# WeeFav/Visual-Odometry-GPU

Measured on AMD Instinct MI355X. Metric: ORB detect+describe frames/sec (1241x376, 8 lvls), higher is better.
Workload: dtype u8; 1 GPU; KITTI-shaped 1241x376 u8, 8 levels s=1.2, 1000 features, FAST-9 t=20, NMS 3x3, Harris top-N, blur5 all levels, BRIEF-256; batch=1024 frames/step/GPU resident in HBM (stream A); distinct_resident_batches=2, fast_early_exit=True, pyramid_blur_fused=True, pyramid_top_rows_first=True, pipelined_batches=True

## Files before the change

### visual-odometry-gpu_amd/csrc/orbx_kernels.hip

```cpp
#include <hip/hip_runtime.h>

#include <cstdlib>

#include "orbx_internal.h"
#include "orbx_math.h"
#include "orbx_wave.h"

__constant__ __attribute__((aligned(16))) int8_t c_pattern[1024] = {
#include "pattern_31.inc"
};


typedef uint16_t __attribute__((aligned(1))) u16_unaligned;

__device__ __forceinline__ void decode_tile(const OrbxTileMap& tm, int nlevels, int& l, int& tx, int& ty) {
  const int t = blockIdx.x;
  l = 0;
#pragma unroll 1
  for (int i = 1; i < nlevels; i++)
    if (t >= tm.begin[i]) l = i;
  const int local = t - tm.begin[l];
  ty = local / tm.tiles_x[l];
  tx = local - ty * tm.tiles_x[l];
}

__device__ __forceinline__ int reflect101(int p, int len) {
  if (p < 0) p = -p;
  if (p >= len) p = 2 * len - p - 2;
  p = p < 0 ? 0 : p;
  return p >= len ? len - 1 : p;
}

typedef uint32_t __attribute__((aligned(1))) u32_unaligned;
struct __attribute__((packed, aligned(1))) uint2_unaligned {
  uint32_t x, y;
  __device__ operator uint2() const { return make_uint2(x, y); }
};

template <int ROWS, bool WIN8>
__device__ __forceinline__ void pyr_rows(const uint8_t* __restrict__ src, int in_stride, int w0, int h0,
                                         const OrbxResizeTap* __restrict__ ytaps, int yb, int lh,
                                         const uint32_t (&ofs)[4], const uint32_t (&cc)[4],
                                         __amdgpu_buffer_rsrc_t rout, uint32_t voff_st, uint32_t vmask, int pitch) {
// ... 320 lines not shown
    for (int j = 0; j < K; j++) out[j] = pr[j] + 2.0f * pr[j + 1] + pr[j + 2];
  };
  float pr[3][P], hs[3][K];
  cvt_row(0, pr[0]);
  cvt_row(1, pr[1]);
  hsum(pr[0], hs[0]);
  hsum(pr[1], hs[1]);
  float a = 0.f, b = 0.f, c = 0.f;
#pragma unroll
  for (int i = 0; i < K; i++) {
    float(&p0)[P] = pr[i % 3];
    float(&p1)[P] = pr[(i + 1) % 3];
    float(&p2)[P] = pr[(i + 2) % 3];
    cvt_row(i + 2, p2);
    hsum(p2, hs[(i + 2) % 3]);
    float vs[P];
#pragma unroll
    for (int j = 0; j < P; j++) vs[j] = p0[j] + 2.0f * p1[j] + p2[j];
#pragma unroll
    for (int j = 0; j < K; j++) {
      const float gx = vs[j + 2] - vs[j];
      const float gy = hs[(i + 2) % 3][j] - hs[i % 3][j];
      const float wgt = g[i * K + j];
      a = __fadd_rn(a, __fmul_rn(__fmul_rn(gx, gx), wgt));
      c = __fadd_rn(c, __fmul_rn(__fmul_rn(gy, gy), wgt));
      b = __fadd_rn(b, __fmul_rn(__fmul_rn(gx, gy), wgt));
    }
  }
  const float det = __fsub_rn(__fmul_rn(a, c), __fmul_rn(b, b));
  const float trace = __fadd_rn(a, c);
  return __fsub_rn(det, __fmul_rn(__fmul_rn(kk, trace), trace));
}

__device__ __forceinline__ float harris_any(const uint8_t* img, int w, int h, int pitch, int x, int y,
                                            const float* __restrict__ g, int K, float kk) {
  const int m = K / 2 + 1;
  if (x >= m - 1 && y >= m - 1 && x <= w - m && y <= h - m && w >= 4 && h >= 4) {
    if (K == 7) return harris_fast<7>(img, w, h, pitch, x, y, g, kk);
    if (K == 5) return harris_fast<5>(img, w, h, pitch, x, y, g, kk);
    if (K == 3) return harris_fast<3>(img, w, h, pitch, x, y, g, kk);
  }
  return harris_at(img, w, h, pitch, x, y, g, K, kk);
}

template <int K, int RPL, int G>
__device__ __forceinline__ float harris_row_group(const uint8_t* img, int pitch, int x, int y,
                                                  const float* __restrict__ g, float kk, int sub) {
  constexpr int r = K / 2, P = K + 2, NR = RPL + 2;
  constexpr int NL = (K + RPL - 1) / RPL;
  const int row0 = (sub < NL ? sub : NL - 1) * RPL;
  const int xs = x - r - 1;
  const int a0 = xs & ~3, off = xs - a0;
  float p[NR][P];
#pragma unroll
  for (int i = 0; i < NR; i++) {
    const int pr = min(row0 + i, P - 1);
    const uint32_t* row = reinterpret_cast<const uint32_t*>(img + (size_t)(y - r - 1 + pr) * pitch + a0);
    const uint32_t d0 = row[0], d1 = row[1], d2 = row[2];
    const uint32_t q[3] = {__builtin_amdgcn_alignbyte(d1, d0, off), __builtin_amdgcn_alignbyte(d2, d1, off),
                           d2 >> (8 * off)};
#pragma unroll
    for (int j = 0; j < P; j++) p[i][j] = (float)((q[j >> 2] >> (8 * (j & 3))) & 0xffu);
  }
  float hs[NR][K];
#pragma unroll
  for (int i = 0; i < NR; i++)
#pragma unroll
    for (int j = 0; j < K; j++) hs[i][j] = p[i][j] + 2.0f * p[i][j + 1] + p[i][j + 2];
  float pa[RPL][K], pb[RPL][K], pc[RPL][K];
#pragma unroll
// ... 63 lines not shown
      last = (5 + RPL - 1) / RPL - 1;
    } else {
      v = harris_row_group<3, RPL, G>(img, pitch, xx, yy, g, kk, sub);
      last = (3 + RPL - 1) / RPL - 1;
    }
    if (active && fast && sub == last) {
      res = v;
      writer = true;
    }
  }
  if (active && !fast && sub == 0) {
    res = harris_at(img, w, h, pitch, x, y, g, K, kk);
    writer = true;
  }
  return res;
}

__global__ __launch_bounds__(256) void k_harris2_flat(const uint8_t* __restrict__ img, int w, int h, int pitch,
                                                      const orbx_keypoint* __restrict__ kps, int nkp,
                                                      const float* __restrict__ gauss, int K, float kk,
                                                      float* __restrict__ resp) {
  constexpr int G = 8, RPL = 1;
  const int j = blockIdx.x * 32 + (threadIdx.x >> 3), sub = threadIdx.x & 7;
  const bool active = j < nkp;
  orbx_keypoint kp = {4, 4};
  if (active) kp = kps[j];
  bool writer;
  const float v = harris_group<RPL, G>(img, w, h, pitch, kp.x, kp.y, gauss, K, kk, sub, active, writer);
  if (writer) resp[j] = v;
}


#define LVL_THREADS 512
__global__ __launch_bounds__(LVL_THREADS) __attribute__((amdgpu_waves_per_eu(4, 8))) void k_level_select(OrbxPlan plan, int mode, const u64* __restrict__ mask,
                                                              const uint8_t* __restrict__ pyr,
                                                              const float* __restrict__ gauss, int K, float kk,
                                                              orbx_keypoint* __restrict__ sel_lkp,
                                                              float* __restrict__ sel_resp,
                                                              int32_t* __restrict__ sel_count,
                                                              uint32_t* __restrict__ need) {
  extern __shared__ __attribute__((aligned(16))) unsigned char s_dyn[];
  __shared__ int s_wsum[4][LVL_THREADS / 64];
  const int f = blockIdx.x, l = blockIdx.y;
  const OrbxLevel& L = plan.L[l];
  const int cap = L.cap, cap2 = (cap + 1) & ~1;
  u64* s_key = reinterpret_cast<u64*>(s_dyn);
  uint32_t* s_kp = reinterpret_cast<uint32_t*>(s_dyn + 8 * (size_t)cap2);
  float* s_r = reinterpret_cast<float*>(s_dyn + 12 * (size_t)cap2);
  const u64* m = mask + (size_t)f * plan.mask_words + L.mask_off;
  const int nwords = L.h * L.mask_wpr;
  const int tid = threadIdx.x, lane = tid & 63, wave = tid >> 6;

  int base = 0;
  for (int w0 = 0; w0 < nwords && base < cap; w0 += 4 * LVL_THREADS) {
    u64 v[4];
#pragma unroll
    for (int q = 0; q < 4; q++) {
      const int i = w0 + LVL_THREADS * q + tid;
      v[q] = i < nwords ? m[i] : 0ull;
    }
    int incl[4], c[4];
#pragma unroll
    for (int q = 0; q < 4; q++) {
      c[q] = __popcll(v[q]);
      incl[q] = wave_scan_incl(c[q]);
      if (lane == 63) s_wsum[q][wave] = incl[q];
    }
    __syncthreads();
#pragma unroll
    for (int q = 0; q < 4; q++) {
      int woff = 0, tot = 0;
#pragma unroll
      for (int k = 0; k < LVL_THREADS / 64; k++) {
        const int sv = s_wsum[q][k];
        if (k < wave) woff += sv;
        tot += sv;
      }
      int pos = base + woff + incl[q] - c[q];
      if (c[q] && pos < cap) {
        const int i = w0 + LVL_THREADS * q + tid;
        const int y = i / L.mask_wpr, xw = i - y * L.mask_wpr;
        u64 w = v[q];
        while (w && pos < cap) {
          const int b = __ffsll((long long)w) - 1;
          w &= w - 1;
          s_kp[pos++] = ((uint32_t)y << 16) | (uint32_t)orbx_mask_x(L, xw, b);
        }
      }
      base += tot;
    }
    __syncthreads();
  }
  const int n = base < cap ? base : cap;
  const int keep = n < L.quota ? n : L.quota;
  const size_t so = (size_t)f * plan.out_cap + L.out_off;
  if (tid == 0) sel_count[f * plan.nlevels + l] = keep;
  if (need && tid == 0 && cap > 0) atomicMax(&need[l], base >= cap ? (s_kp[cap - 1] >> 16) + 1u : (uint32_t)L.h);

  if (mode == ORBX_SELECT_ROWMAJOR) {
    for (int i = tid; i < keep; i += LVL_THREADS) {
      const uint32_t p = s_kp[i];
      orbx_keypoint kp;
      kp.x = (int)(p & 0xffffu);
      kp.y = (int)(p >> 16);
      sel_lkp[so + i] = kp;
      sel_resp[so + i] = 0.0f;
    }
    return;
  }

  const uint8_t* img = pyr + (size_t)f * plan.frame_bytes + L.img_off;
  const int n2 = (n + 1) & ~1;
  for (int i = tid; i < n2; i += LVL_THREADS) {
    u64 key = 0ull;
    if (i < n) {
      const uint32_t p = s_kp[i];
      const float r = harris_any(img, L.w, L.h, L.pitch, (int)(p & 0xffffu), (int)(p >> 16), gauss, K, kk);
      s_r[i] = r;
      uint32_t u = orbx_f2u(r);
      if (u == 0x80000000u) u = 0u;
      u ^= (u >> 31) ? 0xffffffffu : 0x80000000u;
      key = ((u64)u << 32) | (uint32_t)~(uint32_t)i;
    }
    s_key[i] = key;
  }
  __syncthreads();

  for (int i = tid; i < n; i += LVL_THREADS) {
    const u64 ki = s_key[i];
    int rank = 0;
#pragma unroll 4
    for (int j = 0; j < n2; j += 2) {
      const ulonglong2 v = *reinterpret_cast<const ulonglong2*>(&s_key[j]);
      rank += v.x > ki;
      rank += v.y > ki;
    }
    if (rank < keep) {
      const uint32_t p = s_kp[i];
      orbx_keypoint kp;
      kp.x = (int)(p & 0xffffu);
      kp.y = (int)(p >> 16);
      sel_lkp[so + rank] = kp;
      sel_resp[so + rank] = s_r[i];
    }
  }
}

__global__ __launch_bounds__(256) void k_lvl_compact(OrbxPlan plan, const u64* __restrict__ mask,
                                                     uint32_t* __restrict__ cand, int32_t* __restrict__ ncand,
                                                     uint32_t* __restrict__ need) {
  __shared__ int s_wsum[4][4];
  const int l = blockIdx.x, f = blockIdx.y;
  const OrbxLevel& L = plan.L[l];
  const int cap = L.cap;
  const u64* m = mask + (size_t)f * plan.mask_words + L.mask_off;
  uint32_t* out = cand + (size_t)f * plan.cand_total + L.cand_off;
  const int nwords = L.h * L.mask_wpr;
  const int tid = threadIdx.x, lane = tid & 63, wave = tid >> 6;
  int base = 0;
  for (int w0 = 0; w0 < nwords && base < cap; w0 += 1024) {
    u64 v[4];
#pragma unroll
    for (int q = 0; q < 4; q++) {
      const int i = w0 + 256 * q + tid;
      v[q] = i < nwords ? m[i] : 0ull;
    }
    int incl[4], c[4];
#pragma unroll
    for (int q = 0; q < 4; q++) {
      c[q] = __popcll(v[q]);
      incl[q] = wave_scan_incl(c[q]);
      if (lane == 63) s_wsum[q][wave] = incl[q];
    }
    __syncthreads();
#pragma unroll
    for (int q = 0; q < 4; q++) {
// ... 265 lines not shown



#define DESC_NLD ((DESC_ROWS * (DESC_PITCH / 4) + 63) / 64)

__device__ __forceinline__ void desc_fetch_patch(const DescJob& jb, int lane, uint32_t (&regs)[DESC_NLD],
                                                 int& off_out) {
  const int px0 = jb.x - DESC_R, py0 = jb.y - DESC_R;
  const int ax0 = px0 & ~3;
  off_out = px0 - ax0;
  int row = lane / (DESC_PITCH / 4), c = lane - row * (DESC_PITCH / 4);
#pragma unroll
  for (int k = 0; k < DESC_NLD; k++) {
    const int gy = py0 + row, gx = ax0 + 4 * c;
    uint32_t v = 0;
    if (lane + 64 * k < DESC_ROWS * (DESC_PITCH / 4) && (unsigned)gy < (unsigned)jb.h &&
        (unsigned)gx < (unsigned)jb.pitch)
      v = *reinterpret_cast<const uint32_t*>(jb.img + (uint32_t)(gy * jb.pitch + gx));
    regs[k] = v;
    row += 5;
    c += 4;
    if (c >= DESC_PITCH / 4) {
      c -= DESC_PITCH / 4;
      row += 1;
    }
  }
}

struct DescLds2 {
  uint32_t patch[DESC_ROWS * DESC_PITCH / 4];
  uint16_t hs[DESC_ROWS * DESC_HP];
};

template <class L>
__device__ __forceinline__ void desc_store_patch(L& lds, int lane, const uint32_t (&regs)[DESC_NLD]) {
#pragma unroll
  for (int k = 0; k < DESC_NLD; k++)
    if (lane + 64 * k < DESC_ROWS * (DESC_PITCH / 4)) lds.patch[lane + 64 * k] = regs[k];
}

__device__ __forceinline__ DescJob desc_job(const OrbxPlan& plan, const uint8_t* pyr, int f, orbx_keypoint kp,
                                            int level) {
  const OrbxLevel& L = plan.L[level];
  DescJob jb;
  jb.img = pyr + (size_t)f * plan.frame_bytes + L.img_off;
  jb.w = L.w;
  jb.h = L.h;
  jb.pitch = L.pitch;
  jb.x = kp.x;
  jb.y = kp.y;
  jb.valid = true;
  return jb;
}

template <class L>
__device__ __forceinline__ void desc_box_table_fused(L& lds, int lane) {
  static_assert(DESC_BROWS == 37, "6 chunks: 7 + 5 x 6 rows");
  const int chunk = lane / 10, g = lane - chunk * 10;
  if (chunk < 6) {
    const int r0 = chunk == 0 ? 0 : 6 * chunk + 1, nrows = chunk == 0 ? 7 : 6;
    const uint32_t* pp = &lds.patch[r0 * (DESC_PITCH / 4) + g];
    uint2* bp = reinterpret_cast<uint2*>(&lds.hs[r0 * DESC_HP + 4 * g]);
    auto hrow = [&](int i) {
      const u64 v = hsum5x4(pp[i * (DESC_PITCH / 4)], pp[i * (DESC_PITCH / 4) + 1]);
      return make_uint2((uint32_t)v, (uint32_t)(v >> 32));
    };
// ... 2 lines not shown
    for (int i = 0; i < 5; i++) q[i] = hrow(i);
    uint2 acc;
    acc.x = pk_add(pk_add(pk_add(q[0].x, q[1].x), pk_add(q[2].x, q[3].x)), q[4].x);
    acc.y = pk_add(pk_add(pk_add(q[0].y, q[1].y), pk_add(q[2].y, q[3].y)), q[4].y);
    bp[0] = acc;
#pragma unroll
    for (int i = 1; i < 7; i++) {
      if (i < nrows) {
        const uint2 nw = hrow(i + 4);
        const uint2 od = q[(i - 1) % 5];
        acc.x = pk_sub(pk_add(acc.x, nw.x), od.x);
        acc.y = pk_sub(pk_add(acc.y, nw.y), od.y);
        q[(i - 1) % 5] = nw;
        bp[i * (DESC_HP / 4)] = acc;
      }
    }
  }
  wave_lds_sync();
}

__device__ __forceinline__ float lround_f(float v) {
  const float t = __builtin_truncf(v);
  const float fr = __fsub_rn(v, t);
  return __fadd_rn(t, __builtin_truncf(__fadd_rn(fr, fr)));
}

typedef float f2_t __attribute__((ext_vector_type(2)));
typedef int i2_t __attribute__((ext_vector_type(2)));
__device__ __forceinline__ i2_t lround_small2(f2_t v) {
  const f2_t h = {0.5f - 0x1p-25f, 0.5f - 0x1p-25f};
  return __builtin_convertvector(v + __builtin_elementwise_copysign(h, v), i2_t);
}

template <int DESC_KPW, int DESC_NW, int DESC_OCC>
__global__ __launch_bounds__(64 * DESC_NW, DESC_OCC) void k_describe2(OrbxPlan plan, const uint8_t* __restrict__ pyr, int patch_size,
                                                   const int32_t* __restrict__ sel_count,
                                                   const orbx_keypoint* __restrict__ sel_lkp,
                                                   const float* __restrict__ sel_resp,
                                                   int32_t* __restrict__ out_count,
                                                   orbx_keypoint* __restrict__ out_lkp,
                                                   float* __restrict__ out_resp,
                                                   int32_t* __restrict__ out_level,
                                                   orbx_keypoint* __restrict__ out_kp,
                                                   uint32_t* __restrict__ out_kp16,
                                                   float* __restrict__ out_angle,
                                                   orbx_descriptor* __restrict__ out_desc,
                                                   const uint32_t* __restrict__ feedback, uint32_t* __restrict__ feedback_host,
                                                   OrbxHostRecord host) {
  constexpr int DESC_KPB = DESC_NW * DESC_KPW;
  static_assert(2 * DESC_KPB <= 64 * DESC_NW, "trig: two threads per keypoint");
  __shared__ __attribute__((aligned(16))) DescLds2 s_lds[DESC_NW];
  __shared__ int s_m[DESC_KPB][2];
  __shared__ float s_cs[DESC_KPB][2];
  __shared__ uint2 s_mw[4 * (DESC_PITCH / 4)];
  __shared__ __attribute__((aligned(16))) uint32_t s_rec_kp[DESC_KPB], s_rec_angle[DESC_KPB], s_rec_desc[DESC_KPB][8];
  const int f = blockIdx.x, grp = blockIdx.y, tid = threadIdx.x, lane = tid & 63;
  const int wave = __builtin_amdgcn_readfirstlane(tid >> 6);
  static_assert(ORBX_MAX_LEVELS <= 64, "one lane per level");
  const int lvl_cnt = lane < plan.nlevels ? sel_count[f * plan.nlevels + lane] : 0;
  const int lvl_end = wave_scan_incl(lvl_cnt);
  const int count = __builtin_amdgcn_readlane(lvl_end, 63);
  if (grp == 0 && tid == 0) {
    out_count[f] = count;
    if (host.counts) host.counts[f] = count;
  }
  if (feedback_host && grp == 0 && f == 0 && tid < ORBX_FEEDBACK_WORDS) feedback_host[tid] = feedback[tid];
  const int slot0 = grp * DESC_KPB;
  if (slot0 >= count) return;
  DescLds2& lds = s_lds[wave];
  const int pr = patch_size / 2;
  if (tid < 4 * (DESC_PITCH / 4)) {
    const int off = tid / (DESC_PITCH / 4), c = tid - off * (DESC_PITCH / 4);
    uint32_t xw = 0, on = 0;
#pragma unroll
    for (int b = 0; b < 4; b++) {
      const int t = 4 * c + b - off - (DESC_R - pr);
      if (t >= 0 && t <= 2 * pr) {
        xw |= (uint32_t)t << (8 * b);
        on |= 1u << (8 * b);
      }
    }
    s_mw[tid] = make_uint2(xw, on);
  }
  int rowk[DESC_NLD], c3[3];
  uint32_t rin = 0;
  {
    int row = lane / (DESC_PITCH / 4), c = lane - row * (DESC_PITCH / 4);
#pragma unroll
    for (int k = 0; k < DESC_NLD; k++) {
      rowk[k] = row;
      __builtin_assume(row >= 0 && row < DESC_ROWS + 6);
      if (k < 3) c3[k] = c;
      if (lane + 64 * k < DESC_ROWS * (DESC_PITCH / 4) && row >= DESC_R - pr && row <= DESC_R + pr) rin |= 1u << k;
      row += 5;
      c += 4;
      if (c >= DESC_PITCH / 4) {
        c -= DESC_PITCH / 4;
        row += 1;
      }
    }
  }
  __syncthreads();
  const size_t fo = (size_t)f * plan.out_cap;

  const int nk = min(DESC_KPW, max(0, count - (slot0 + wave * DESC_KPW)));
  DescJob jobs[DESC_KPW];
  float scale[DESC_KPW];
  uint32_t regs[DESC_KPW][DESC_NLD];
  int offs[DESC_KPW];
#pragma unroll
  for (int j = 0; j < DESC_KPW; j++) {
    const int slot = min(slot0 + wave * DESC_KPW + j, count - 1);
    const int level = __popcll(__ballot(lvl_end <= slot));
    const int lvl_begin = __builtin_amdgcn_readlane(lvl_end - lvl_cnt, level);
    const size_t src = fo + plan.L[level].out_off + (slot - lvl_begin);
    const orbx_keypoint kp = sel_lkp[src];
    jobs[j] = desc_job(plan, pyr, f, kp, level);
    scale[j] = plan.L[level].scale;
    if (j < nk && lane == 0) {
      out_lkp[fo + slot] = kp;
      out_resp[fo + slot] = sel_resp[src];
      out_level[fo + slot] = level;
    }
  }
#pragma unroll
  for (int j = 0; j < DESC_KPW; j++) {
    const DescJob& jb = jobs[j];
    const int py0 = jb.y - DESC_R, ax0 = (jb.x - DESC_R) & ~3;
    if (py0 >= 0 && py0 + DESC_ROWS <= jb.h && ax0 >= 0 && ax0 + DESC_PITCH <= jb.pitch) {
      offs[j] = jb.x - DESC_R - ax0;
      const uint32_t base = (uint32_t)(py0 * jb.pitch + ax0);
#pragma unroll
      for (int k = 0; k < DESC_NLD; k++) {
        regs[j][k] = 0;
        if (lane + 64 * k < DESC_ROWS * (DESC_PITCH / 4))
          regs[j][k] = *reinterpret_cast<const uint32_t*>(jb.img + (base + (__umul24((uint32_t)rowk[k], (uint32_t)jb.pitch) + 4u * (uint32_t)c3[k % 3])));
      }
    } else {
      desc_fetch_patch(jb, lane, regs[j], offs[j]);
    }
  }

  int pm[2][DESC_KPW];
#pragma unroll
  for (int j = 0; j < DESC_KPW; j++) {
    const DescJob& jb = jobs[j];
    const int off = offs[j];
    pm[0][j] = pm[1][j] = 0;
    if (j < nk && !(jb.x - pr < 0 || jb.x + pr >= jb.w || jb.y - pr < 0 || jb.y + pr >= jb.h)) {
      uint2 mw[3];
#pragma unroll
      for (int m = 0; m < 3; m++) mw[m] = s_mw[off * (DESC_PITCH / 4) + c3[m]];
      uint32_t X = 0, S = 0, M = 0;
#pragma unroll
      for (int k = 0; k < DESC_NLD; k++) {
        const uint32_t z = regs[j][k] & (uint32_t)(-(int32_t)((rin >> k) & 1u));
        X = __builtin_amdgcn_udot4(z, mw[k % 3].x, X, false);
        const uint32_t rs = __builtin_amdgcn_udot4(z, mw[k % 3].y, 0u, false);
        S += rs;
        M += __umul24((uint32_t)rowk[k], rs);
      }
      pm[0][j] = (int)X - __mul24(pr, (int)S);
      pm[1][j] = (int)M - __mul24(DESC_R, (int)S);
    }
  }
  if constexpr (DESC_KPW == 4) {
    int u[2];
#pragma unroll
    for (int i = 0; i < 2; i++) {
      const auto h0 = __builtin_amdgcn_permlane32_swap(pm[i][0], pm[i][1], false, false);
      const auto h1 = __builtin_amdgcn_permlane32_swap(pm[i][2], pm[i][3], false, false);
      const auto r = __builtin_amdgcn_permlane16_swap(h0[0] + h0[1], h1[0] + h1[1], false, false);
      u[i] = row_sum16(r[0] + r[1]);
    }
    if ((lane & 15) == 0) {
      const int q = wave * DESC_KPW + (((lane >> 4) & 1) << 1 | (lane >> 5));
      s_m[q][0] = u[0];
      s_m[q][1] = u[1];
    }
  } else {
#pragma unroll
    for (int j = 0; j < DESC_KPW; j++) {
      const int m10 = wave_sum(pm[0][j]), m01 = wave_sum(pm[1][j]);
      if (lane == 0) {
        s_m[wave * DESC_KPW + j][0] = m10;
        s_m[wave * DESC_KPW + j][1] = m01;
      }
    }
  }
  __syncthreads();
  if (tid < 2 * DESC_KPB && slot0 + (tid >> 1) < count) {
    const int q = tid >> 1, want_sin = tid & 1;
    const float angle = orbx_atan2f((float)s_m[q][1], (float)s_m[q][0]);
    s_cs[q][want_sin] = orbx_sincosf_impl(angle, want_sin ^ 1);
    if (!want_sin) {
      out_angle[fo + slot0 + q] = angle;
      s_rec_angle[q] = __float_as_uint(angle);
    }
  }
  __syncthreads();

  f2_t patx[4], paty[4];
#pragma unroll
  for (int k = 0; k < 4; k++) {
    const int32_t pk = reinterpret_cast<const int32_t*>(c_pattern)[k * 64 + lane];
    patx[k] = f2_t{(float)(int8_t)(pk & 0xff), (float)(int8_t)((pk >> 16) & 0xff)};
    paty[k] = f2_t{(float)(int8_t)((pk >> 8) & 0xff), (float)(int8_t)((pk >> 24) & 0xff)};
  }
#pragma unroll
  for (int j = 0; j < DESC_KPW; j++) {
    if (j < nk) {
      const DescJob& jb = jobs[j];
      const int q = wave * DESC_KPW + j, off = offs[j];
      desc_store_patch(lds, lane, regs[j]);
      wave_lds_sync();
      desc_box_table_fused(lds, lane);
      const float c = s_cs[q][0], s = s_cs[q][1];
      const bool interior = jb.x >= DESC_R && jb.y >= DESC_R && jb.x < jb.w - DESC_R && jb.y < jb.h - DESC_R;
      u64 d[4];
      if (interior) {
        const uint16_t* tbl = &lds.hs[18 * DESC_HP + 18 + off];
        auto at = [&](int x, int y) {
          int i = __mul24(y, DESC_HP) + x;
          asm("" : "+v"(i));
          return tbl[i];
        };
        const f2_t C2 = {c, c}, S2 = {s, s};
#pragma unroll
        for (int k = 0; k < 4; k++) {
          const f2_t X = patx[k], Y = paty[k];
          const i2_t rx = lround_small2(C2 * X - S2 * Y), ry = lround_small2(S2 * X + C2 * Y);
          d[k] = __ballot(at(rx.x, ry.x) < at(rx.y, ry.y));
        }
      } else {
#pragma unroll
        for (int k = 0; k < 4; k++) {
          const float x1 = patx[k].x, y1 = paty[k].x, x2 = patx[k].y, y2 = paty[k].y;
          const int dx1 = orbx_lroundf(__fsub_rn(__fmul_rn(c, x1), __fmul_rn(s, y1)));
          const int dy1 = orbx_lroundf(__fadd_rn(__fmul_rn(s, x1), __fmul_rn(c, y1)));
          const int dx2 = orbx_lroundf(__fsub_rn(__fmul_rn(c, x2), __fmul_rn(s, y2)));
          const int dy2 = orbx_lroundf(__fadd_rn(__fmul_rn(s, x2), __fmul_rn(c, y2)));
          const int cx1 = jb.x + dx1, cy1 = jb.y + dy1, cx2 = jb.x + dx2, cy2 = jb.y + dy2;
          const bool ok = !(cx1 < 2 || cy1 < 2 || cx1 > jb.w - 1 || cy1 > jb.h - 1 || cx2 < 2 || cy2 < 2 ||
                            cx2 > jb.w - 1 || cy2 > jb.h - 1);
          const int s1 = lds.hs[(dy1 + 18) * DESC_HP + dx1 + 18 + off];
          const int s2 = lds.hs[(dy2 + 18) * DESC_HP + dx2 + 18 + off];
          d[k] = __ballot(ok && s1 < s2);
// ... 163 lines not shown

#define ORBX_LAUNCH_CHECK() hipGetLastError()

hipError_t orbx_launch_pyramid2(hipStream_t s, const OrbxTileDesc* d_tiles, int n_tiles, int frame_bytes, int w0,
                                int h0, int n_frames, const uint8_t* d_in, int in_stride, size_t in_frame_stride,
                                const OrbxResizeTap* d_taps, uint8_t* d_pyr) {
  if (n_tiles <= 0) return hipSuccess;
  dim3 grid(n_tiles | 1, n_frames);
  hipLaunchKernelGGL(k_pyramid2, grid, dim3(256), 0, s, d_tiles, n_tiles, frame_bytes, w0, h0, d_in, in_stride,
                     in_frame_stride, d_taps, d_pyr);
  return ORBX_LAUNCH_CHECK();
}

hipError_t orbx_launch_blur(hipStream_t s, const OrbxPlan& plan, const OrbxTileMap& tm, int n_frames,
                            const uint8_t* d_src, uint8_t* d_dst, int first_level, int kind) {
  dim3 grid(tm.begin[plan.nlevels], n_frames);
  hipLaunchKernelGGL(k_blur, grid, dim3(256), 0, s, plan, tm, d_src, d_dst, first_level, kind);
  return ORBX_LAUNCH_CHECK();
}

hipError_t orbx_launch_compact(hipStream_t s, const OrbxPlan& plan, int n_frames,
                               const unsigned long long* d_mask, orbx_keypoint* d_cand, int32_t* d_cand_count,
                               int32_t* d_cand_total, int need_total) {
  dim3 grid(plan.nlevels, n_frames);
  hipLaunchKernelGGL(k_compact, grid, dim3(256), 0, s, plan, d_mask, d_cand, d_cand_count, d_cand_total,
                     need_total);
  return ORBX_LAUNCH_CHECK();
}

hipError_t orbx_launch_level_select(hipStream_t s, const OrbxPlan& plan, int n_frames, int mode,
                                    const unsigned long long* d_mask, const uint8_t* d_pyr, const float* d_gauss,
                                    int window, float k, orbx_keypoint* d_sel_lkp, float* d_sel_resp,
                                    int32_t* d_sel_count, uint32_t* d_need) {
  int maxcap = 2;
  for (int l = 0; l < plan.nlevels; l++) maxcap = plan.L[l].cap > maxcap ? plan.L[l].cap : maxcap;
  const size_t lds = (size_t)((maxcap + 1) & ~1) * 16;
  dim3 grid(n_frames, plan.nlevels);
  hipLaunchKernelGGL(k_level_select, grid, dim3(LVL_THREADS), lds, s, plan, mode, d_mask, d_pyr, d_gauss, window, k,
                     d_sel_lkp, d_sel_resp, d_sel_count, d_need);
  return ORBX_LAUNCH_CHECK();
}

hipError_t orbx_launch_level_select_auto(hipStream_t s, const OrbxPlan& plan, int n_frames, int mode, int force,
                                         const unsigned long long* d_mask, const uint8_t* d_pyr,
                                         const float* d_gauss, int window, float k, uint32_t* d_cand,
                                         int32_t* d_ncand, float* d_cresp, orbx_keypoint* d_sel_lkp,
                                         float* d_sel_resp, int32_t* d_sel_count, uint32_t* d_need) {
  int maxcap = 2;
  for (int l = 0; l < plan.nlevels; l++) maxcap = plan.L[l].cap > maxcap ? plan.L[l].cap : maxcap;
  const bool spread = mode == ORBX_SELECT_HARRIS &&
                      (force >= 0 ? force != 0 : maxcap > LVL_THREADS);
  if (!spread)
    return orbx_launch_level_select(s, plan, n_frames, mode, d_mask, d_pyr, d_gauss, window, k, d_sel_lkp,
                                    d_sel_resp, d_sel_count, d_need);
  hipLaunchKernelGGL(k_lvl_compact, dim3(plan.nlevels, n_frames), dim3(256), 0, s, plan, d_mask, d_cand, d_ncand, d_need);
  hipLaunchKernelGGL(k_lvl_harris, dim3((maxcap + 255) / 256, plan.nlevels, n_frames), dim3(256), 0, s, plan, d_pyr,
                     d_gauss, window, k, d_cand, d_ncand, d_cresp);
  const size_t lds = (size_t)((maxcap + 7) & ~7) * 8;
  hipLaunchKernelGGL(k_lvl_rank, dim3((maxcap + RANK_SLICE - 1) / RANK_SLICE, plan.nlevels, n_frames), dim3(256), lds,
                     s, plan, d_cand, d_ncand, d_cresp, d_sel_lkp, d_sel_resp, d_sel_count);
  return ORBX_LAUNCH_CHECK();
}

hipError_t orbx_launch_describe(hipStream_t s, const OrbxPlan& plan, int n_frames, const uint8_t* d_pyr,
                                int patch_size, const int32_t* d_sel_count, const orbx_keypoint* d_sel_lkp,
                                const float* d_sel_resp, int32_t* d_out_count, orbx_keypoint* d_out_lkp,
                                float* d_out_resp, int32_t* d_out_level, orbx_keypoint* d_out_kp, uint32_t* d_out_kp16,
                                float* d_out_angle, orbx_descriptor* d_out_desc, const uint32_t* d_feedback,
                                uint32_t* h_feedback, const OrbxHostRecord* host_record) {
  const OrbxHostRecord host = host_record ? *host_record : OrbxHostRecord{};
  if (plan.out_cap <= 0) return hipSuccess;
  if ((long long)plan.out_cap * n_frames <= 8192) {
    dim3 grid(n_frames, (plan.out_cap + 3) / 4);
    hipLaunchKernelGGL((k_describe2<1, 4, 1>), grid, dim3(256), 0, s, plan, d_pyr, patch_size, d_sel_count, d_sel_lkp,
                       d_sel_resp, d_out_count, d_out_lkp, d_out_resp, d_out_level, d_out_kp, d_out_kp16, d_out_angle, d_out_desc, d_feedback,
                       h_feedback, host);
  } else {
    dim3 grid(n_frames, (plan.out_cap + 15) / 16);
    hipLaunchKernelGGL((k_describe2<4, 4, 6>), grid, dim3(256), 0, s, plan, d_pyr, patch_size, d_sel_count, d_sel_lkp,
                       d_sel_resp, d_out_count, d_out_lkp, d_out_resp, d_out_level, d_out_kp, d_out_kp16, d_out_angle, d_out_desc, d_feedback,
                       h_feedback, host);
  }
  return ORBX_LAUNCH_CHECK();
}

hipError_t orbx_launch_describe_flat(hipStream_t s, const uint8_t* d_img, int w, int h, int pitch,
                                     const orbx_keypoint* d_kps, int nkp, int patch_size, int use_given_angles,
                                     int do_brief, float* d_angles, orbx_descriptor* d_desc) {
  if (nkp <= 0) return hipSuccess;
  hipLaunchKernelGGL(k_describe_flat, dim3((nkp + 3) / 4), dim3(256), 0, s, d_img, w, h, pitch, d_kps, nkp,
                     patch_size, use_given_angles, do_brief, d_angles, d_desc);
  return ORBX_LAUNCH_CHECK();
}

hipError_t orbx_launch_harris_flat(hipStream_t s, const uint8_t* d_img, int w, int h, int pitch,
                                   const orbx_keypoint* d_kps, int nkp, const float* d_gauss, int K, float kk,
                                   float* d_resp) {
  if (nkp <= 0) return hipSuccess;
  hipLaunchKernelGGL(k_harris2_flat, dim3((nkp + 31) / 32), dim3(256), 0, s, d_img, w, h, pitch, d_kps, nkp,
                     d_gauss, K, kk, d_resp);
  return ORBX_LAUNCH_CHECK();
}

hipError_t orbx_launch_nms_f32(hipStream_t s, const float* d_scores, int w, int h, int radius, float threshold,
                               unsigned long long* d_mask, int mask_wpr) {
  dim3 grid((w + 63) / 64, (h + 3) / 4);
  hipLaunchKernelGGL(k_nms_f32, grid, dim3(256), 0, s, d_scores, w, h, radius, threshold, d_mask, mask_wpr);
  return ORBX_LAUNCH_CHECK();
}

hipError_t orbx_launch_conv2d(hipStream_t s, const uint8_t* d_img, int w, int h, int pitch, const float* d_kernel,
                              int K, int reflect_pad, uint8_t* d_dst, int dst_pitch) {
// ... 26 lines not shown
```

Measured before the change: 552,200 frames/s.

## Specialize describe kernel for 31-pixel patches with per-lane row-run patch loads

Adds a patch_size==31 specialization of the describe kernel. Each lane now loads contiguous row runs from a compile-time constant table (5+2+1 words), so the image-moment computation needs fewer dot products and no per-word row masking or row multiply. The BRIEF pattern is also precomputed as floats in constant memory, removing per-lane int8 unpacking and conversion. The cost is an extra template instantiation, added register and constant-memory footprint, and a hand-built lane mapping that has to cover the patch correctly.

```diff
diff --git a/visual-odometry-gpu_amd/csrc/orbx_desc_layout.h b/visual-odometry-gpu_amd/csrc/orbx_desc_layout.h
--- /dev/null
+++ b/visual-odometry-gpu_amd/csrc/orbx_desc_layout.h
@@ -0,0 +1,26 @@
+#pragma once
+
+#define DESC31_NA 5
+#define DESC31_NB 2
+
+struct Desc31Run {
+  int row, col;
+};
+
+constexpr Desc31Run desc31_pair(int p) {
+  if (p < 31) return Desc31Run{5 + p, 10};
+  if (p == 31) return Desc31Run{0, 10};
+  const int q = p - 32, r = q / 6;
+  return Desc31Run{r < 4 ? 1 + r : 36 + (r - 4), 2 * (q - 6 * r)};
+}
+
+constexpr Desc31Run desc31_run_a(int lane) {
+  return lane < 62 ? Desc31Run{5 + (lane >> 1), 5 * (lane & 1)} : Desc31Run{0, 5 * (lane - 62)};
+}
+constexpr Desc31Run desc31_run_b(int lane) { return desc31_pair(lane); }
+constexpr Desc31Run desc31_run_c(int lane) {
+  if (lane >= 44) return desc31_pair(lane);
+  const Desc31Run p = desc31_pair(64 + (lane >> 1));
+  return Desc31Run{p.row, p.col + (lane & 1)};
+}
+constexpr int desc31_wcol(int lane) { return lane < 62 ? 5 * (lane & 1) : 11; }
diff --git a/visual-odometry-gpu_amd/csrc/orbx_kernels.hip b/visual-odometry-gpu_amd/csrc/orbx_kernels.hip
--- a/visual-odometry-gpu_amd/csrc/orbx_kernels.hip
+++ b/visual-odometry-gpu_amd/csrc/orbx_kernels.hip
@@ -2,6 +2,7 @@
 
 #include <cstdlib>
 
+#include "orbx_desc_layout.h"
 #include "orbx_internal.h"
 #include "orbx_math.h"
 #include "orbx_wave.h"
@@ -9,6 +10,24 @@
 __constant__ __attribute__((aligned(16))) int8_t c_pattern[1024] = {
 #include "pattern_31.inc"
 };
+
+struct DescPatternF {
+  float v[4][64][4];
+};
+constexpr DescPatternF desc_pattern_f() {
+  constexpr int8_t p[1024] = {
+#include "pattern_31.inc"
+  };
+  DescPatternF t{};
+  for (int i = 0; i < 256; i++) {
+    t.v[i / 64][i % 64][0] = p[4 * i];
+    t.v[i / 64][i % 64][1] = p[4 * i + 2];
+    t.v[i / 64][i % 64][2] = p[4 * i + 1];
+    t.v[i / 64][i % 64][3] = p[4 * i + 3];
+  }
+  return t;
+}
+__constant__ __attribute__((aligned(16))) DescPatternF c_pattern_f = desc_pattern_f();
 
 
 typedef uint16_t __attribute__((aligned(1))) u16_unaligned;
@@ -969,6 +988,24 @@
   uint16_t hs[DESC_ROWS * DESC_HP];
 };
 
+struct Desc31Lane {
+  int ra, rb, rc, wa;
+  uint32_t oa, ob, oc, pad;
+};
+struct Desc31Table {
+  Desc31Lane l[64];
+};
+constexpr Desc31Table desc31_table() {
+  Desc31Table t{};
+  for (int lane = 0; lane < 64; lane++) {
+    const Desc31Run a = desc31_run_a(lane), b = desc31_run_b(lane), c = desc31_run_c(lane);
+    t.l[lane] = Desc31Lane{a.row, b.row, c.row, desc31_wcol(lane), (uint32_t)(a.row * DESC_PITCH + 4 * a.col),
+                           (uint32_t)(b.row * DESC_PITCH + 4 * b.col), (uint32_t)(c.row * DESC_PITCH + 4 * c.col), 0u};
+  }
+  return t;
+}
+__constant__ __attribute__((aligned(16))) Desc31Table c_desc31 = desc31_table();
+
 template <class L>
 __device__ __forceinline__ void desc_store_patch(L& lds, int lane, const uint32_t (&regs)[DESC_NLD]) {
 #pragma unroll
@@ -1037,7 +1074,7 @@
   return __builtin_convertvector(v + __builtin_elementwise_copysign(h, v), i2_t);
 }
 
-template <int DESC_KPW, int DESC_NW, int DESC_OCC>
+template <int DESC_KPW, int DESC_NW, int DESC_OCC, bool DESC_P31>
 __global__ __launch_bounds__(64 * DESC_NW, DESC_OCC) void k_describe2(OrbxPlan plan, const uint8_t* __restrict__ pyr, int patch_size,
                                                    const int32_t* __restrict__ sel_count,
                                                    const orbx_keypoint* __restrict__ sel_lkp,
@@ -1057,7 +1094,7 @@
   __shared__ __attribute__((aligned(16))) DescLds2 s_lds[DESC_NW];
   __shared__ int s_m[DESC_KPB][2];
   __shared__ float s_cs[DESC_KPB][2];
-  __shared__ uint2 s_mw[4 * (DESC_PITCH / 4)];
+  __shared__ uint2 s_mw[4 * 16];
   __shared__ __attribute__((aligned(16))) uint32_t s_rec_kp[DESC_KPB], s_rec_angle[DESC_KPB], s_rec_desc[DESC_KPB][8];
   const int f = blockIdx.x, grp = blockIdx.y, tid = threadIdx.x, lane = tid & 63;
   const int wave = __builtin_amdgcn_readfirstlane(tid >> 6);
@@ -1073,9 +1110,9 @@
   const int slot0 = grp * DESC_KPB;
   if (slot0 >= count) return;
   DescLds2& lds = s_lds[wave];
-  const int pr = patch_size / 2;
-  if (tid < 4 * (DESC_PITCH / 4)) {
-    const int off = tid / (DESC_PITCH / 4), c = tid - off * (DESC_PITCH / 4);
+  const int pr = DESC_P31 ? 15 : patch_size / 2;
+  if (tid < 4 * 16) {
+    const int off = tid / 16, c = tid - off * 16;
     uint32_t xw = 0, on = 0;
 #pragma unroll
     for (int b = 0; b < 4; b++) {
@@ -1089,7 +1126,10 @@
   }
   int rowk[DESC_NLD], c3[3];
   uint32_t rin = 0;
-  {
+  Desc31Lane ly{};
+  if constexpr (DESC_P31) {
+    ly = c_desc31.l[lane];
+  } else {
     int row = lane / (DESC_PITCH / 4), c = lane - row * (DESC_PITCH / 4);
 #pragma unroll
     for (int k = 0; k < DESC_NLD; k++) {
@@ -1132,7 +1172,34 @@
   for (int j = 0; j < DESC_KPW; j++) {
     const DescJob& jb = jobs[j];
     const int py0 = jb.y - DESC_R, ax0 = (jb.x - DESC_R) & ~3;
-    if (py0 >= 0 && py0 + DESC_ROWS <= jb.h && ax0 >= 0 && ax0 + DESC_PITCH <= jb.pitch) {
+    const bool inside = py0 >= 0 && py0 + DESC_ROWS <= jb.h && ax0 >= 0 && ax0 + DESC_PITCH <= jb.pitch;
+    if constexpr (DESC_P31) {
+      offs[j] = jb.x - DESC_R - ax0;
+      if (inside) {
+        const uint8_t* img = jb.img + (uint32_t)(py0 * jb.pitch + ax0);
+        const uint32_t dp = (uint32_t)(jb.pitch - DESC_PITCH);
+        const uint32_t* pa = reinterpret_cast<const uint32_t*>(img + (__umul24((uint32_t)ly.ra, dp) + ly.oa));
+        const uint32_t* pb = reinterpret_cast<const uint32_t*>(img + (__umul24((uint32_t)ly.rb, dp) + ly.ob));
+        const uint32_t* pc = reinterpret_cast<const uint32_t*>(img + (__umul24((uint32_t)ly.rc, dp) + ly.oc));
+#pragma unroll
+        for (int k = 0; k < DESC31_NA; k++) regs[j][k] = pa[k];
+#pragma unroll
+        for (int k = 0; k < DESC31_NB; k++) regs[j][DESC31_NA + k] = pb[k];
+        regs[j][DESC_NLD - 1] = pc[0];
+      } else {
+        auto ld = [&](int row, uint32_t o) -> uint32_t {
+          const int gy = py0 + row, gx = ax0 + (int)o - row * DESC_PITCH;
+          return (unsigned)gy < (unsigned)jb.h && (unsigned)gx < (unsigned)jb.pitch
+                     ? *reinterpret_cast<const uint32_t*>(jb.img + (uint32_t)(gy * jb.pitch + gx))
+                     : 0u;
+        };
+#pragma unroll
+        for (int k = 0; k < DESC31_NA; k++) regs[j][k] = ld(ly.ra, ly.oa + 4 * k);
+#pragma unroll
+        for (int k = 0; k < DESC31_NB; k++) regs[j][DESC31_NA + k] = ld(ly.rb, ly.ob + 4 * k);
+        regs[j][DESC_NLD - 1] = ld(ly.rc, ly.oc);
+      }
+    } else if (inside) {
       offs[j] = jb.x - DESC_R - ax0;
       const uint32_t base = (uint32_t)(py0 * jb.pitch + ax0);
 #pragma unroll
@@ -1153,20 +1220,32 @@
     const int off = offs[j];
     pm[0][j] = pm[1][j] = 0;
     if (j < nk && !(jb.x - pr < 0 || jb.x + pr >= jb.w || jb.y - pr < 0 || jb.y + pr >= jb.h)) {
-      uint2 mw[3];
-#pragma unroll
-      for (int m = 0; m < 3; m++) mw[m] = s_mw[off * (DESC_PITCH / 4) + c3[m]];
-      uint32_t X = 0, S = 0, M = 0;
-#pragma unroll
-      for (int k = 0; k < DESC_NLD; k++) {
-        const uint32_t z = regs[j][k] & (uint32_t)(-(int32_t)((rin >> k) & 1u));
-        X = __builtin_amdgcn_udot4(z, mw[k % 3].x, X, false);
-        const uint32_t rs = __builtin_amdgcn_udot4(z, mw[k % 3].y, 0u, false);
-        S += rs;
-        M += __umul24((uint32_t)rowk[k], rs);
-      }
-      pm[0][j] = (int)X - __mul24(pr, (int)S);
-      pm[1][j] = (int)M - __mul24(DESC_R, (int)S);
+      if constexpr (DESC_P31) {
+        const uint2* mw = &s_mw[off * 16 + ly.wa];
+        uint32_t X = 0, S = 0;
+#pragma unroll
+        for (int k = 0; k < DESC31_NA; k++) {
+          X = __builtin_amdgcn_udot4(regs[j][k], mw[k].x, X, false);
+          S = __builtin_amdgcn_udot4(regs[j][k], mw[k].y, S, false);
+        }
+        pm[0][j] = (int)X - __mul24(pr, (int)S);
+        pm[1][j] = __mul24(ly.ra - DESC_R, (int)S);
+      } else {
+        uint2 mw[3];
+#pragma unroll
+        for (int m = 0; m < 3; m++) mw[m] = s_mw[off * 16 + c3[m]];
+        uint32_t X = 0, S = 0, M = 0;
+#pragma unroll
+        for (int k = 0; k < DESC_NLD; k++) {
+          const uint32_t z = regs[j][k] & (uint32_t)(-(int32_t)((rin >> k) & 1u));
+          X = __builtin_amdgcn_udot4(z, mw[k % 3].x, X, false);
+          const uint32_t rs = __builtin_amdgcn_udot4(z, mw[k % 3].y, 0u, false);
+          S += rs;
+          M += __umul24((uint32_t)rowk[k], rs);
+        }
+        pm[0][j] = (int)X - __mul24(pr, (int)S);
+        pm[1][j] = (int)M - __mul24(DESC_R, (int)S);
+      }
     }
   }
   if constexpr (DESC_KPW == 4) {
@@ -1208,16 +1287,27 @@
   f2_t patx[4], paty[4];
 #pragma unroll
   for (int k = 0; k < 4; k++) {
-    const int32_t pk = reinterpret_cast<const int32_t*>(c_pattern)[k * 64 + lane];
-    patx[k] = f2_t{(float)(int8_t)(pk & 0xff), (float)(int8_t)((pk >> 16) & 0xff)};
-    paty[k] = f2_t{(float)(int8_t)((pk >> 8) & 0xff), (float)(int8_t)((pk >> 24) & 0xff)};
+    const float4 v = *reinterpret_cast<const float4*>(c_pattern_f.v[k][lane]);
+    patx[k] = f2_t{v.x, v.y};
+    paty[k] = f2_t{v.z, v.w};
   }
 #pragma unroll
   for (int j = 0; j < DESC_KPW; j++) {
     if (j < nk) {
       const DescJob& jb = jobs[j];
       const int q = wave * DESC_KPW + j, off = offs[j];
-      desc_store_patch(lds, lane, regs[j]);
+      if constexpr (DESC_P31) {
+        uint32_t* pa = reinterpret_cast<uint32_t*>(reinterpret_cast<uint8_t*>(lds.patch) + ly.oa);
+        uint32_t* pb = reinterpret_cast<uint32_t*>(reinterpret_cast<uint8_t*>(lds.patch) + ly.ob);
+        uint32_t* pc = reinterpret_cast<uint32_t*>(reinterpret_cast<uint8_t*>(lds.patch) + ly.oc);
+#pragma unroll
+        for (int k = 0; k < DESC31_NA; k++) pa[k] = regs[j][k];
+#pragma unroll
+        for (int k = 0; k < DESC31_NB; k++) pb[k] = regs[j][DESC31_NA + k];
+        pc[0] = regs[j][DESC_NLD - 1];
+      } else {
+        desc_store_patch(lds, lane, regs[j]);
+      }
       wave_lds_sync();
       desc_box_table_fused(lds, lane);
       const float c = s_cs[q][0], s = s_cs[q][1];
@@ -1485,14 +1575,17 @@
                                 uint32_t* h_feedback, const OrbxHostRecord* host_record) {
   const OrbxHostRecord host = host_record ? *host_record : OrbxHostRecord{};
   if (plan.out_cap <= 0) return hipSuccess;
+  const bool p31 = patch_size == 31;
   if ((long long)plan.out_cap * n_frames <= 8192) {
     dim3 grid(n_frames, (plan.out_cap + 3) / 4);
-    hipLaunchKernelGGL((k_describe2<1, 4, 1>), grid, dim3(256), 0, s, plan, d_pyr, patch_size, d_sel_count, d_sel_lkp,
+    auto* kern = p31 ? k_describe2<1, 4, 1, true> : k_describe2<1, 4, 1, false>;
+    hipLaunchKernelGGL(kern, grid, dim3(256), 0, s, plan, d_pyr, patch_size, d_sel_count, d_sel_lkp,
                        d_sel_resp, d_out_count, d_out_lkp, d_out_resp, d_out_level, d_out_kp, d_out_kp16, d_out_angle, d_out_desc, d_feedback,
                        h_feedback, host);
   } else {
     dim3 grid(n_frames, (plan.out_cap + 15) / 16);
-    hipLaunchKernelGGL((k_describe2<4, 4, 6>), grid, dim3(256), 0, s, plan, d_pyr, patch_size, d_sel_count, d_sel_lkp,
+    auto* kern = p31 ? k_describe2<4, 4, 6, true> : k_describe2<4, 4, 6, false>;
+    hipLaunchKernelGGL(kern, grid, dim3(256), 0, s, plan, d_pyr, patch_size, d_sel_count, d_sel_lkp,
                        d_sel_resp, d_out_count, d_out_lkp, d_out_resp, d_out_level, d_out_kp, d_out_kp16, d_out_angle, d_out_desc, d_feedback,
                        h_feedback, host);
   }
```

After: 550,300 frames/s (median of 2 runs). About the same (-0.3%).

## Restructure level select: wave-per-level compaction, multi-level blocks, sorted-run ranking

Applied to the files above, without the earlier changes.

Rewrites the level-select kernel so one block handles all pyramid levels of a frame when the batch is large. Each level is compacted by a single wave, without block-wide barriers. Harris responses are computed in 64-wide runs, with a specialised fast-path template on the window size. Each run is sorted with a wave bitonic sort, and ranks come from binary searches across the other runs instead of an O(n^2) all-pairs comparison. This cuts barriers, launch granularity and ranking cost, but adds LDS pressure from holding every level's slots. Plans needing more than 4096 slots now fall back to the spread path.

```diff
diff --git a/visual-odometry-gpu_amd/csrc/orbx_kernels.hip b/visual-odometry-gpu_amd/csrc/orbx_kernels.hip
--- a/visual-odometry-gpu_amd/csrc/orbx_kernels.hip
+++ b/visual-odometry-gpu_amd/csrc/orbx_kernels.hip
@@ -395,10 +395,14 @@
   return __fsub_rn(det, __fmul_rn(__fmul_rn(kk, trace), trace));
 }
 
+__device__ __forceinline__ bool harris_fast_ok(int w, int h, int x, int y, int K) {
+  const int m = K / 2 + 1;
+  return x >= m - 1 && y >= m - 1 && x <= w - m && y <= h - m && w >= 4 && h >= 4;
+}
+
 __device__ __forceinline__ float harris_any(const uint8_t* img, int w, int h, int pitch, int x, int y,
                                             const float* __restrict__ g, int K, float kk) {
-  const int m = K / 2 + 1;
-  if (x >= m - 1 && y >= m - 1 && x <= w - m && y <= h - m && w >= 4 && h >= 4) {
+  if (harris_fast_ok(w, h, x, y, K)) {
     if (K == 7) return harris_fast<7>(img, w, h, pitch, x, y, g, kk);
     if (K == 5) return harris_fast<5>(img, w, h, pitch, x, y, g, kk);
     if (K == 3) return harris_fast<3>(img, w, h, pitch, x, y, g, kk);
@@ -528,116 +532,189 @@
 
 
 #define LVL_THREADS 512
-__global__ __launch_bounds__(LVL_THREADS) __attribute__((amdgpu_waves_per_eu(4, 8))) void k_level_select(OrbxPlan plan, int mode, const u64* __restrict__ mask,
-                                                              const uint8_t* __restrict__ pyr,
-                                                              const float* __restrict__ gauss, int K, float kk,
-                                                              orbx_keypoint* __restrict__ sel_lkp,
-                                                              float* __restrict__ sel_resp,
-                                                              int32_t* __restrict__ sel_count,
-                                                              uint32_t* __restrict__ need) {
+#define LVL_WAVES (LVL_THREADS / 64)
+#define LVL_Q 16
+#define LVL_RUN 64
+#define LVL_MAX_SLOTS 4096
+
+__host__ __device__ inline int lvl_slots(const OrbxPlan& plan, int nl) {
+  int s = 0;
+  for (int l = 0; l < nl; l++) s += (plan.L[l].cap + LVL_RUN - 1) & ~(LVL_RUN - 1);
+  return s;
+}
+
+__device__ __forceinline__ u64 shfl_xor_u64(u64 v, int m) {
+  const int lo = __shfl_xor((int)(uint32_t)v, m), hi = __shfl_xor((int)(uint32_t)(v >> 32), m);
+  return ((u64)(uint32_t)hi << 32) | (uint32_t)lo;
+}
+
+__device__ __forceinline__ u64 wave_sort_desc(u64 k, int lane) {
+#pragma unroll
+  for (int b = 2; b <= 64; b <<= 1)
+#pragma unroll
+    for (int j = b >> 1; j > 0; j >>= 1) {
+      const u64 o = shfl_xor_u64(k, j);
+      const bool keep_max = ((lane & j) == 0) == ((lane & b) == 0);
+      k = keep_max ? (o > k ? o : k) : (o < k ? o : k);
+    }
+  return k;
+}
+
+__device__ __forceinline__ int lvl_of_run(const int* s_runs, int l0, int l1, int& r) {
+  int l = l0;
+  while (l < l1 - 1) {
+    const int c = __builtin_amdgcn_readfirstlane(s_runs[l]);
+    if (r < c) break;
+    r -= c;
+    l++;
+  }
+  return l;
+}
+
+template <int KF>
+__global__ __launch_bounds__(LVL_THREADS) __attribute__((amdgpu_waves_per_eu(4, 8))) void k_level_select(
+    OrbxPlan plan, int lpg, int mode, const u64* __restrict__ mask, const uint8_t* __restrict__ pyr,
+    const float* __restrict__ gauss, int K, float kk, orbx_keypoint* __restrict__ sel_lkp,
+    float* __restrict__ sel_resp, int32_t* __restrict__ sel_count, uint32_t* __restrict__ need) {
   extern __shared__ __attribute__((aligned(16))) unsigned char s_dyn[];
-  __shared__ int s_wsum[4][LVL_THREADS / 64];
-  const int f = blockIdx.x, l = blockIdx.y;
-  const OrbxLevel& L = plan.L[l];
-  const int cap = L.cap, cap2 = (cap + 1) & ~1;
+  __shared__ int s_n[ORBX_MAX_LEVELS];
+  __shared__ int s_runs[ORBX_MAX_LEVELS];
+  const int f = blockIdx.x, nl = plan.nlevels;
+  const int l0 = blockIdx.y * lpg, l1 = min(l0 + lpg, nl);
+  const int nslots = lvl_slots(plan, nl);
   u64* s_key = reinterpret_cast<u64*>(s_dyn);
-  uint32_t* s_kp = reinterpret_cast<uint32_t*>(s_dyn + 8 * (size_t)cap2);
-  float* s_r = reinterpret_cast<float*>(s_dyn + 12 * (size_t)cap2);
-  const u64* m = mask + (size_t)f * plan.mask_words + L.mask_off;
-  const int nwords = L.h * L.mask_wpr;
-  const int tid = threadIdx.x, lane = tid & 63, wave = tid >> 6;
-
-  int base = 0;
-  for (int w0 = 0; w0 < nwords && base < cap; w0 += 4 * LVL_THREADS) {
-    u64 v[4];
-#pragma unroll
-    for (int q = 0; q < 4; q++) {
-      const int i = w0 + LVL_THREADS * q + tid;
-      v[q] = i < nwords ? m[i] : 0ull;
-    }
-    int incl[4], c[4];
-#pragma unroll
-    for (int q = 0; q < 4; q++) {
-      c[q] = __popcll(v[q]);
-      incl[q] = wave_scan_incl(c[q]);
-      if (lane == 63) s_wsum[q][wave] = incl[q];
-    }
-    __syncthreads();
-#pragma unroll
-    for (int q = 0; q < 4; q++) {
-      int woff = 0, tot = 0;
-#pragma unroll
-      for (int k = 0; k < LVL_THREADS / 64; k++) {
-        const int sv = s_wsum[q][k];
-        if (k < wave) woff += sv;
-        tot += sv;
-      }
-      int pos = base + woff + incl[q] - c[q];
-      if (c[q] && pos < cap) {
-        const int i = w0 + LVL_THREADS * q + tid;
-        const int y = i / L.mask_wpr, xw = i - y * L.mask_wpr;
-        u64 w = v[q];
-        while (w && pos < cap) {
-          const int b = __ffsll((long long)w) - 1;
-          w &= w - 1;
-          s_kp[pos++] = ((uint32_t)y << 16) | (uint32_t)orbx_mask_x(L, xw, b);
+  uint32_t* s_kp = reinterpret_cast<uint32_t*>(s_dyn + 8 * (size_t)nslots);
+  float* s_r = reinterpret_cast<float*>(s_dyn + 12 * (size_t)nslots);
+  const int tid = threadIdx.x, lane = tid & 63;
+  const int wave = __builtin_amdgcn_readfirstlane(tid >> 6);
+  const size_t fo = (size_t)f * plan.out_cap;
+
+  for (int l = l0 + wave; l < l1; l += LVL_WAVES) {
+    const OrbxLevel& L = plan.L[l];
+    const int cap = L.cap, slot = lvl_slots(plan, l);
+    const u64* m = mask + (size_t)f * plan.mask_words + L.mask_off;
+    const int nwords = L.h * L.mask_wpr;
+    int base = 0, last = -1;
+    for (int w0 = 0; w0 < nwords && base < cap; w0 += 64 * LVL_Q) {
+      u64 v[LVL_Q];
+#pragma unroll
+      for (int q = 0; q < LVL_Q; q++) {
+        const int i = w0 + 64 * q + lane;
+        v[q] = i < nwords ? m[i] : 0ull;
+      }
+#pragma unroll
+      for (int q = 0; q < LVL_Q; q++) {
+        const int c = __popcll(v[q]);
+        const int incl = wave_scan_incl(c);
+        int pos = base + incl - c;
+        if (c && pos < cap) {
+          const int i = w0 + 64 * q + lane;
+          const int y = i / L.mask_wpr, xw = i - y * L.mask_wpr;
+          u64 w = v[q];
+          while (w && pos < cap) {
+            const int b = __ffsll((long long)w) - 1;
+            w &= w - 1;
+            const int x = orbx_mask_x(L, xw, b);
+            if (mode == ORBX_SELECT_ROWMAJOR) {
+              orbx_keypoint kp;
+              kp.x = x;
+              kp.y = y;
+              sel_lkp[fo + L.out_off + pos] = kp;
+              sel_resp[fo + L.out_off + pos] = 0.0f;
+            } else {
+              s_kp[slot + pos] = ((uint32_t)y << 16) | (uint32_t)x;
+            }
+            if (pos == cap - 1) last = y;
+            pos++;
+          }
         }
-      }
-      base += tot;
-    }
-    __syncthreads();
-  }
-  const int n = base < cap ? base : cap;
-  const int keep = n < L.quota ? n : L.quota;
-  const size_t so = (size_t)f * plan.out_cap + L.out_off;
-  if (tid == 0) sel_count[f * plan.nlevels + l] = keep;
-  if (need && tid == 0 && cap > 0) atomicMax(&need[l], base >= cap ? (s_kp[cap - 1] >> 16) + 1u : (uint32_t)L.h);
-
-  if (mode == ORBX_SELECT_ROWMAJOR) {
-    for (int i = tid; i < keep; i += LVL_THREADS) {
-      const uint32_t p = s_kp[i];
+        base += __builtin_amdgcn_readlane(incl, 63);
+      }
+    }
+    const int n = base < cap ? base : cap;
+    const int keep = n < L.quota ? n : L.quota;
+    const int runs = (n + LVL_RUN - 1) / LVL_RUN;
+    const u64 found = __ballot(last >= 0);
+    const int last_row = found ? __builtin_amdgcn_readlane(last, __ffsll((long long)found) - 1) : L.h - 1;
+    if (lane == 0) {
+      s_n[l] = n;
+      s_runs[l] = runs;
+      sel_count[f * nl + l] = keep;
+      if (need && cap > 0) atomicMax(&need[l], (uint32_t)last_row + 1u);
+    }
+  }
+  if (mode == ORBX_SELECT_ROWMAJOR) return;
+  __syncthreads();
+
+  int nruns = 0;
+  for (int l = l0; l < l1; l++) nruns += s_runs[l];
+  nruns = __builtin_amdgcn_readfirstlane(nruns);
+  const uint8_t* img_f = pyr + (size_t)f * plan.frame_bytes;
+  if (KF > 0) {
+    for (int t = wave; t < nruns; t += LVL_WAVES) {
+      int r = t;
+      const int l = lvl_of_run(s_runs, l0, l1, r);
+      const OrbxLevel& L = plan.L[l];
+      const int slot = lvl_slots(plan, l), i = LVL_RUN * r + lane;
+      const bool live = i < __builtin_amdgcn_readfirstlane(s_n[l]);
+      const uint32_t p = live ? s_kp[slot + i] : 0u;
+      const int x = (int)(p & 0xffffu), y = (int)(p >> 16);
+      const bool fast = live && harris_fast_ok(L.w, L.h, x, y, KF);
+      if (fast) s_r[slot + i] = harris_fast<KF>(img_f + L.img_off, L.w, L.h, L.pitch, x, y, gauss, kk);
+    }
+  }
+  for (int t = wave; t < nruns; t += LVL_WAVES) {
+    int r = t;
+    const int l = lvl_of_run(s_runs, l0, l1, r);
+    const OrbxLevel& L = plan.L[l];
+    const int slot = lvl_slots(plan, l), i = LVL_RUN * r + lane;
+    u64 key = 0ull;
+    if (i < __builtin_amdgcn_readfirstlane(s_n[l])) {
+      const uint32_t p = s_kp[slot + i];
+      const int x = (int)(p & 0xffffu), y = (int)(p >> 16);
+      const bool fast = KF > 0 && harris_fast_ok(L.w, L.h, x, y, KF);
+      float resp;
+      if (fast) {
+        resp = s_r[slot + i];
+      } else {
+        resp = harris_at(img_f + L.img_off, L.w, L.h, L.pitch, x, y, gauss, K, kk);
+        s_r[slot + i] = resp;
+      }
+      uint32_t u = orbx_f2u(resp);
+      if (u == 0x80000000u) u = 0u;
+      u ^= (u >> 31) ? 0xffffffffu : 0x80000000u;
+      key = ((u64)u << 32) | (uint32_t)~(uint32_t)i;
+    }
+    s_key[slot + i] = wave_sort_desc(key, lane);
+  }
+  __syncthreads();
+  for (int t = wave; t < nruns; t += LVL_WAVES) {
+    int r = t;
+    const int l = lvl_of_run(s_runs, l0, l1, r);
+    const int slot = lvl_slots(plan, l);
+    const int runs = __builtin_amdgcn_readfirstlane(s_runs[l]);
+    const u64 k = s_key[slot + LVL_RUN * r + lane];
+    int rank = lane;
+    for (int o = 0; o < runs; o++) {
+      if (o == r) continue;
+      const u64* run = s_key + slot + LVL_RUN * o;
+      int c = 0;
+#pragma unroll
+      for (int step = LVL_RUN / 2; step > 0; step >>= 1) c += run[c + step - 1] > k ? step : 0;
+      c += run[c] > k;
+      rank += c;
+    }
+    const int n = __builtin_amdgcn_readfirstlane(s_n[l]);
+    const int keep = n < plan.L[l].quota ? n : plan.L[l].quota;
+    if (k != 0ull && rank < keep) {
+      const int i = (int)~(uint32_t)k;
+      const uint32_t p = s_kp[slot + i];
       orbx_keypoint kp;
       kp.x = (int)(p & 0xffffu);
       kp.y = (int)(p >> 16);
-      sel_lkp[so + i] = kp;
-      sel_resp[so + i] = 0.0f;
-    }
-    return;
-  }
-
-  const uint8_t* img = pyr + (size_t)f * plan.frame_bytes + L.img_off;
-  const int n2 = (n + 1) & ~1;
-  for (int i = tid; i < n2; i += LVL_THREADS) {
-    u64 key = 0ull;
-    if (i < n) {
-      const uint32_t p = s_kp[i];
-      const float r = harris_any(img, L.w, L.h, L.pitch, (int)(p & 0xffffu), (int)(p >> 16), gauss, K, kk);
-      s_r[i] = r;
-      uint32_t u = orbx_f2u(r);
-      if (u == 0x80000000u) u = 0u;
-      u ^= (u >> 31) ? 0xffffffffu : 0x80000000u;
-      key = ((u64)u << 32) | (uint32_t)~(uint32_t)i;
-    }
-    s_key[i] = key;
-  }
-  __syncthreads();
-
-  for (int i = tid; i < n; i += LVL_THREADS) {
-    const u64 ki = s_key[i];
-    int rank = 0;
-#pragma unroll 4
-    for (int j = 0; j < n2; j += 2) {
-      const ulonglong2 v = *reinterpret_cast<const ulonglong2*>(&s_key[j]);
-      rank += v.x > ki;
-      rank += v.y > ki;
-    }
-    if (rank < keep) {
-      const uint32_t p = s_kp[i];
-      orbx_keypoint kp;
-      kp.x = (int)(p & 0xffffu);
-      kp.y = (int)(p >> 16);
-      sel_lkp[so + rank] = kp;
-      sel_resp[so + rank] = s_r[i];
+      const size_t so = fo + plan.L[l].out_off + rank;
+      sel_lkp[so] = kp;
+      sel_resp[so] = s_r[slot + i];
     }
   }
 }
@@ -1447,12 +1524,15 @@
                                     const unsigned long long* d_mask, const uint8_t* d_pyr, const float* d_gauss,
                                     int window, float k, orbx_keypoint* d_sel_lkp, float* d_sel_resp,
                                     int32_t* d_sel_count, uint32_t* d_need) {
-  int maxcap = 2;
-  for (int l = 0; l < plan.nlevels; l++) maxcap = plan.L[l].cap > maxcap ? plan.L[l].cap : maxcap;
-  const size_t lds = (size_t)((maxcap + 1) & ~1) * 16;
-  dim3 grid(n_frames, plan.nlevels);
-  hipLaunchKernelGGL(k_level_select, grid, dim3(LVL_THREADS), lds, s, plan, mode, d_mask, d_pyr, d_gauss, window, k,
-                     d_sel_lkp, d_sel_resp, d_sel_count, d_need);
+  const int nslots = mode == ORBX_SELECT_ROWMAJOR ? 0 : lvl_slots(plan, plan.nlevels);
+  if (nslots > LVL_MAX_SLOTS) return hipErrorInvalidValue;
+  const size_t lds = (size_t)nslots * 16;
+  const int lpg = n_frames >= 256 ? plan.nlevels : 1;
+  dim3 grid(n_frames, (plan.nlevels + lpg - 1) / lpg);
+  auto kern = window == 7 ? k_level_select<7> : window == 5 ? k_level_select<5> : window == 3 ? k_level_select<3>
+                                                                                   : k_level_select<0>;
+  hipLaunchKernelGGL(kern, grid, dim3(LVL_THREADS), lds, s, plan, lpg, mode, d_mask, d_pyr, d_gauss, window, k, d_sel_lkp,
+                     d_sel_resp, d_sel_count, d_need);
   return ORBX_LAUNCH_CHECK();
 }
 
@@ -1464,7 +1544,8 @@
   int maxcap = 2;
   for (int l = 0; l < plan.nlevels; l++) maxcap = plan.L[l].cap > maxcap ? plan.L[l].cap : maxcap;
   const bool spread = mode == ORBX_SELECT_HARRIS &&
-                      (force >= 0 ? force != 0 : maxcap > LVL_THREADS);
+                      (lvl_slots(plan, plan.nlevels) > LVL_MAX_SLOTS ||
+                       (force >= 0 ? force != 0 : maxcap > LVL_THREADS));
   if (!spread)
     return orbx_launch_level_select(s, plan, n_frames, mode, d_mask, d_pyr, d_gauss, window, k, d_sel_lkp,
                                     d_sel_resp, d_sel_count, d_need);
```

After: 558,900 frames/s before, 579,800 frames/s after (median of 6 runs). +3.7%, better.
